# godhj93/bayesian-torch

Hardware: AMD Instinct MI355X
Metric: MC-samples/sec (forward+KL), Bayesian-ResNet18 CIFAR batch=128 (higher is better)
Workload: dtype f32 (bf16x3 split operands, 6 product terms, f32 accumulate); 1 GPU; cfg3: Bayesian-ResNet18 via dnn_to_bnn (Conv2dReparameterization), CIFAR 3x32x32, batch=128; samples_per_launch=32, batch=128, rng=on-chip philox, parallelism=mc1, output_stage=bn+relu+residual (+ the stem max-pool) folded into the conv kernels, launch=hip graph replay

## Files before the change

### bayesian_torch_amd/csrc/bt_fused_fwd.h

```cpp
#pragma once
#include <type_traits>

#include "bt_api_internal.h"

namespace bt {

typedef float f32x16 __attribute__((ext_vector_type(16)));

constexpr int kBK = 36;
constexpr int kMaxTaps = 128;
#ifndef BT_STAMPS
#define BT_STAMPS 0
#endif
constexpr bool kStamps = BT_STAMPS != 0;
constexpr int kThreads = 512;
constexpr int kProducers = 256;

struct FwdArgs {
  const float *x, *mu_w, *rho_w, *mu_b, *rho_b, *pmu_w, *psig_w, *pmu_b, *psig_b;
  const float *mu_pk, *sig_pk;
  const float *eps_w, *eps_b, *sign_in, *sign_out;
  float* out;
  float* kl_out;
  double* slots;
  unsigned* counter;
  long long x_sample_stride, x_elems, out_elems, w_elems;
  int B, Ci, H, W, Co, KH, KW, SH, SW, PH, PW, DH, DW, G;
  int Ho, Wo, HoWo, M, K, Cig, Cog, S, T, HW;
  int n_tiles, m_tiles, total_blocks;
  int t_NI, t_R, t_Wt, n_bt, n_rt, n_ct;
  int patch_ok;
  int x_cvec;
  int x_rows;
  int pixel_major, mt_per_pixel;
  int w_vec, x_vec;
  int do_kl, kl_slices;
  uint32_t seed_lo, seed_hi, call, layer_id, sample0;
  const uint32_t* call_base;
  const float *ep_scale, *ep_shift, *ep_res;
  long long ep_res_stride;
  int ep_relu;
  int ep_pool, ep_Hp, ep_Wp;
  int out_vec4;
  int bn32;
  unsigned long long* dbg;
  uint32_t inv_m_tiles, inv_S, inv_n_tiles, inv_n_bt, inv_n_ct, inv_rw, inv_wt, inv_kw;
  int x_flat;
  int row_taps;
  float* sk_scratch;
  unsigned* sk_tickets;
  long long sk_scratch_bytes;
  int sk_nsl, sk_ks, sk_cpt;
  int sk_kh0, sk_nh, sk_kw0, sk_nw;
  int d_tap;
};

__device__ __forceinline__ int xcd_remap(int orig, int n) {
  const int q = n >> 3, r = n & 7, xcd = orig & 7, i = orig >> 3;
  return (xcd < r ? xcd * (q + 1) : r * (q + 1) + (xcd - r) * q) + i;
}

__host__ __device__ inline int row_chunks(int x_lo, int x_hi, int W, int* xa_out) {
  const int xa = x_lo & ~3;
  int n = ((x_hi - xa) >> 2) + 1;
  if (n > 1 && xa + 4 * (n - 1) >= W && xa + 4 <= 0) --n;
  *xa_out = xa;
  return n;
}

template <int BM, bool FLIP = false>
constexpr int x_words() {
  return kBK * ((FLIP && BM > 128 ? 160 : BM <= 256 ? BM : 320) + 1);
}

template <int BN, int BM, bool FLIP>
constexpr int fused_lds_bytes() {
  return (2 * (FLIP ? 2 : 1) * (kBK * (BN + 1) + x_words<BM, FLIP>()) + kMaxTaps * 4 + 24 + 8 + 80) * 4;
}

__device__ __forceinline__ double block_sum_all(double v, double* scratch) {
  v = wave_sum(v);
  const int lane = threadIdx.x & 63, w = threadIdx.x >> 6;
  __syncthreads();
  if (lane == 0) scratch[w] = v;
  __syncthreads();
  double t = 0.0;
  if (threadIdx.x == 0)
// ... 710 lines not shown
```

### bayesian_torch_amd/csrc/bt_fused_split.hip

```cpp
#include <atomic>
#include <stdlib.h>
#include <string.h>

#include "bt_fused_split_quad.h"
#include "bt_fused_split_direct.h"
#include "bt_fused_split_skinny.h"
#include "bt_fused_split_host.h"

namespace bt {

static std::atomic<int> g_contraction{-1};
int contraction_mode() {
  int m = g_contraction.load(std::memory_order_relaxed);
  if (m < 0) {
    const char* e = getenv("BT_CONTRACTION");
    m = !e ? 0 : (!strcmp(e, "f32") ? 1 : !strcmp(e, "bf16x2") ? 2 : 0);
    g_contraction.store(m, std::memory_order_relaxed);
  }
  return m;
}

template <int BM, int NP, int NPW, int XM, int BN = 64>
static int launch_split_cfg(FwdArgs& a, hipStream_t stream) {
  constexpr int lds = split_lds_bytes<BN, BM, NP>();
// ... 6 lines not shown
    if (hipFuncSetAttribute(reinterpret_cast<const void*>(kern), hipFuncAttributeMaxDynamicSharedMemorySize, lds) != hipSuccess)
      return set_error(BT_ERR_HIP_BASE, "fused forward (split): cannot raise the dynamic LDS limit");
    flags[dev] = true;
  }
  char nm[160];
  snprintf(nm, sizeof(nm), "fused_split_kernel<%d,%d,bf16x%d,%d terms,npw=%d,xm=%d>", BN, BM, NP, NP == 3 ? 6 : 3, NPW, XM);
  note_kernel(nm);
  split_fill_inverses(a);
  hipLaunchKernelGGL(kern, dim3((unsigned)a.total_blocks), dim3(256 + 64 * NPW), lds, stream, a);
  return check_launch("fused forward (split)");
}

template <int BM, int NPW>
static int launch_split_xm(FwdArgs& a, int mode, int xm, hipStream_t stream) {
  if (mode == 2) return launch_split_cfg<BM, 2, NPW, 0>(a, stream);
  if constexpr (BM == 128) {
    if (a.bn32) {
      if (xm == 1) return launch_split_cfg<BM, 3, NPW, 1, 32>(a, stream);
      if (xm == 2) return launch_split_cfg<BM, 3, NPW, 2, 32>(a, stream);
      return launch_split_cfg<BM, 3, NPW, 0, 32>(a, stream);
    }
    if (xm == 1) return launch_split_cfg<BM, 3, NPW, 1>(a, stream);
    if (xm == 2) return launch_split_cfg<BM, 3, NPW, 2>(a, stream);
  } else {
    if (xm == 3) return launch_split_cfg<BM, 3, NPW, 3>(a, stream);
    if (xm == 4) return launch_split_cfg<BM, 3, NPW, 4>(a, stream);
    if constexpr (BM == 256) {
      if (xm == 2) return launch_split_cfg<BM, 3, 8, 2>(a, stream);
    }
  }
  return launch_split_cfg<BM, 3, NPW, 0>(a, stream);
}

template <bool POOL>
static int launch_quad_cfg(FwdArgs& a, int mode, hipStream_t stream) {
  constexpr int lds = split_lds_bytes<64, 512, 3>();
  auto launch = [&](auto kern, const char* nm) -> int {
    static bool flags[2][64] = {};
    int dev = 0;
    if (hipGetDevice(&dev) != hipSuccess || dev < 0 || dev >= 64) return set_error(BT_ERR_HIP_BASE, "fused forward (split): hipGetDevice failed");
    if (!flags[mode == 2][dev]) {
      if (hipFuncSetAttribute(reinterpret_cast<const void*>(kern), hipFuncAttributeMaxDynamicSharedMemorySize, lds) != hipSuccess)
        return set_error(BT_ERR_HIP_BASE, "fused forward (split): cannot raise the dynamic LDS limit");
      flags[mode == 2][dev] = true;
    }
    note_kernel(nm);
    split_fill_inverses(a);
    hipLaunchKernelGGL(kern, dim3((unsigned)a.total_blocks), dim3(512), lds, stream, a);
    return check_launch("fused forward (split, quad)");
  };
  return launch(fused_split_quad_kernel<3, POOL>, POOL ? "fused_split_quad_kernel<64,512,bf16x3,6 terms,pool=1>" : "fused_split_quad_kernel<64,512,bf16x3,6 terms,pool=0>");
}

static int launch_quad(FwdArgs& a, int mode, hipStream_t stream) {
  if (a.pixel_major || a.T > 64 || !a.out_vec4 || a.HoWo < 2 || a.Wo > 512) return 1;
  int nh, nw, dys, dxs;
  tap_window(a.KH, a.DH, a.SH, a.PH, a.H, a.Ho, false, &nh, &dys);
  tap_window(a.KW, a.DW, a.SW, a.PW, a.W, a.Wo, false, &nw, &dxs);
  constexpr long long XCAP = kQuadXBytes / 24;
  const long long PWt = (long long)(a.Wo - 1) * (dxs ? a.SW : 1) + dxs + 1;
  int NI, R;
  long long tiles_per_sample;
  if (a.HoWo <= 512) {
    const long long PHt = (long long)(a.Ho - 1) * (dys ? a.SH : 1) + dys + 1;
    NI = 512 / a.HoWo, R = a.Ho;
    if (NI > a.B) NI = a.B;
    while (NI > 1 && NI * PHt * PWt > XCAP) --NI;
    if (NI * PHt * PWt > XCAP) return 1;
    tiles_per_sample = (a.B + NI - 1) / NI;
  } else {
    if (a.ep_pool) return 1;
    NI = 1, R = 512 / a.Wo;
    while (R > 1 && ((long long)(R - 1) * (dys ? a.SH : 1) + dys + 1) * PWt > XCAP) --R;
    if (((long long)(R - 1) * (dys ? a.SH : 1) + dys + 1) * PWt > XCAP) return 1;
    tiles_per_sample = (long long)a.B * ((a.Ho + R - 1) / R);
  }
  if ((double)a.M / ((double)tiles_per_sample * 512) < 0.75) return 1;
  if (a.ep_pool) {
    const int Wp = a.ep_Wp;
    if ((Wp & (Wp - 1)) != 0 || Wp < 4 || Wp > 16 || a.ep_res) return 1;
  }
  a.n_tiles = (a.Cog + 63) / 64;
  a.t_NI = NI, a.t_R = R, a.t_Wt = a.Wo, a.n_bt = (a.B + NI - 1) / NI, a.n_rt = (a.Ho + R - 1) / R, a.n_ct = 1, a.m_tiles = a.n_bt * a.n_rt;
  const long long total = (long long)a.G * a.n_tiles * a.S * a.m_tiles;
  if (total <= 0 || total > 0x7FFFFFFFll) return 1;
  a.total_blocks = (int)total;
  a.kl_slices = total < 256 ? (int)total : 256;
  return a.ep_pool ? launch_quad_cfg<true>(a, mode, stream) : launch_quad_cfg<false>(a, mode, stream);
}

static std::atomic<int> g_bn32{-2};
static std::atomic<int> g_direct_off{0};
static int launch_direct(FwdArgs& a, hipStream_t stream) {
  if (g_direct_off.load(std::memory_order_relaxed)) return 1;
  if (a.ep_pool) return 1;
  if (a.KH == 1 && a.KW == 1 && a.PH == 0 && a.PW == 0) {
    a.d_tap = 0;
  } else if (a.H == 1 && a.W == 1 && a.Ho == 1 && a.Wo == 1 && a.PH % a.DH == 0 && a.PW % a.DW == 0 && a.PH / a.DH < a.KH && a.PW / a.DW < a.KW) {
    a.d_tap = (a.PH / a.DH) * a.KW + a.PW / a.DW;
  } else {
    return 1;
  }
  const bool resident = a.Cig <= kDirectMaxK;
  if ((a.Cig & 63) || (!resident && ((a.Cig % (16 * kDirectChunk)) || a.M < 4096)) || a.M < 64) return 1;
  a.n_tiles = (a.Cog + 63) / 64;
  const long long pairs = (long long)a.G * a.n_tiles * a.S;
  const int nsub = (a.M + 63) / 64;
  static const int wg_env = [] { const char* e = getenv("BT_DIRECT_WGS"); const int v = e ? atoi(e) : 0; return v > 0 ? v : 0; }();
  static const int n_cu = [] { int dev = 0, v = 0; if (hipGetDevice(&dev) != hipSuccess || hipDeviceGetAttribute(&v, hipDeviceAttributeMultiprocessorCount, dev) != hipSuccess || v <= 0) v = 256; return v; }();
  const int wg_target = wg_env ? wg_env : !resident ? n_cu : (a.SH > 1 || a.SW > 1) ? 16 * n_cu : 4 * n_cu;
  long long chunks = (wg_target + pairs - 1) / pairs;
  if (chunks > nsub / 64) chunks = nsub / 64;
  if (chunks < 1) {
    chunks = (256 + pairs - 1) / pairs;
    if (chunks > nsub / 4) chunks = nsub / 4;
    if (chunks < 1) chunks = 1;
  }
  int spc = (int)((nsub + chunks - 1) / chunks);
  if (!resident) spc = (spc + 7) & ~7;
  chunks = (nsub + spc - 1) / spc;
// ... 190 lines not shown
```

### bayesian_torch_amd/csrc/bt_fused_split_host.h

```cpp
#pragma once
#include <stdlib.h>

#include "bt_fused_split.h"

namespace bt {

int contraction_mode();

static inline uint32_t inv_u32(long long d, long long nmax) {
  if (d <= 1 || nmax < 0 || (unsigned long long)nmax * (unsigned long long)d >= (1ull << 32)) return 0u;
  return (uint32_t)(((1ull << 32) + (unsigned long long)d - 1ull) / (unsigned long long)d);
}
static inline void split_fill_inverses(FwdArgs& a) {
  static const bool off = getenv("BT_NO_HOST_INV") != nullptr;
  if (off) {
    a.inv_m_tiles = a.inv_S = a.inv_n_tiles = a.inv_n_bt = a.inv_n_ct = a.inv_rw = a.inv_wt = a.inv_kw = 0u;
    return;
  }
  const long long tb = a.total_blocks;
  a.inv_m_tiles = inv_u32(a.m_tiles, tb);
  a.inv_S = inv_u32(a.S, tb);
  a.inv_n_tiles = inv_u32(a.n_tiles, tb);
  a.inv_n_bt = inv_u32(a.n_bt, a.m_tiles);
  a.inv_n_ct = inv_u32(a.n_ct, a.m_tiles);
  a.inv_rw = inv_u32((long long)a.t_R * a.t_Wt, 1024);
  a.inv_wt = inv_u32(a.t_Wt, 1024);
  a.inv_kw = inv_u32(a.KW, 64);
}

static void tap_window(int K, int D, int S, int P, int In, int Out, bool per_pixel, int* n_act, int* extent, int* n_min = nullptr) {
  int best_n = 0, best_ext = 0, least_n = 1 << 30;
  if (per_pixel) {
    for (int o = 0; o < Out; ++o) {
      int lo = 1 << 30, hi = -1, n = 0;
      for (int k = 0; k < K; ++k)
        if ((unsigned)(o * S - P + k * D) < (unsigned)In) lo = k * D < lo ? k * D : lo, hi = k * D > hi ? k * D : hi, ++n;
      if (n > best_n) best_n = n;
      if (n < least_n) least_n = n;
      if (hi - lo > best_ext) best_ext = hi - lo;
    }
    if (n_min) *n_min = least_n;
  } else {
    int lo = 1 << 30, hi = -1;
    for (int k = 0; k < K; ++k) {
      const int l = P - k * D, c = l > 0 ? (l + S - 1) / S : 0;
      if (c < Out && c * S - l < In) lo = k * D < lo ? k * D : lo, hi = k * D > hi ? k * D : hi, ++best_n;
    }
    best_ext = hi >= lo ? hi - lo : 0;
  }
  *n_act = best_n, *extent = best_ext;
}

static int split_axis_kept(int K, int D, int S, int P, int In, int Out, int* gs_out) {
  int lo = 1 << 30, hi = -1;
  for (int k = 0; k < K; ++k) {
    const int l = P - k * D, c = l > 0 ? (l + S - 1) / S : 0;
    if (c < Out && c * S - l < In) lo = k * D < lo ? k * D : lo, hi = k * D > hi ? k * D : hi;
  }
  *gs_out = 1;
  if (hi < 0) return 0;
// ... 69 lines not shown
```

### bayesian_torch_amd/csrc/bt_fused_split_quad.h

```cpp
#pragma once
#include "bt_fused_split.h"

namespace bt {

constexpr int kQuadXBytes = 2 * split_x_bytes<512, 3>();
constexpr int kQuadXBytesFlip = 38400;
template <bool FLIP>
constexpr int quad_lds_bytes() { return 2 * split_w_bytes<64, 3, FLIP>() + (FLIP ? kQuadXBytesFlip : kQuadXBytes) + kSplitMiscBytes; }

template <int NP, bool POOL, bool FLIP = false>
__global__ __launch_bounds__(512) void fused_split_quad_kernel(const FwdArgs a) {
  constexpr int BN = 64, BM = FLIP ? 256 : 512, kProducers = 256, kThreadsAll = 512, STEPS = kSplitSteps, TPS = 4 * STEPS;
  constexpr int CWM = FLIP ? 2 : 4, CWN = 4 / CWM, WTM = BM / CWM, TN = BN / CWN / 32, TM = WTM / 32, NOP = FLIP ? 2 : 1;
  constexpr int PBQ = 8 * NP;
  constexpr int W_BYTES = split_w_bytes<BN, NP, FLIP>(), W_OP = W_BYTES / NOP, XQ_BYTES = FLIP ? kQuadXBytesFlip : kQuadXBytes;
  constexpr int W_STEP = 2 * NP * BN * 16, W_HALF = NP * BN * 16, W_PIECE = BN * 16;
  constexpr int SROWS = BN, SROW = BM + 4;
  static_assert(!FLIP || NP == 3, "Flipout: the exact split");
  static_assert((4 * BN + NOP * SROWS * SROW) * 4 <= 2 * W_BYTES + XQ_BYTES, "output staging fits the operand buffers");

  extern __shared__ __attribute__((aligned(16))) char smem_c[];
  char* const wbuf = smem_c;
  char* const xq = smem_c + 2 * W_BYTES;
  float* const smem = reinterpret_cast<float*>(smem_c);
  int4* const taptab = reinterpret_cast<int4*>(smem_c + 2 * W_BYTES + XQ_BYTES);
  double* const red = reinterpret_cast<double*>(smem_c + 2 * W_BYTES + XQ_BYTES + kMaxTaps * 16);
  int* const misc = reinterpret_cast<int*>(red + 12);
  int* const eofftab = reinterpret_cast<int*>(taptab + 64);
  (void)red;

  const int tid = threadIdx.x, lane = tid & 63, wave = tid >> 6;
  unsigned long long* const dbg_ = kStamps ? a.dbg : nullptr;
  if (dbg_ && dbg_[201] && tid == 0) {
    dbg_[256 + 4 * blockIdx.x] = __builtin_amdgcn_s_memrealtime();
    dbg_[256 + 4 * blockIdx.x + 2] = __builtin_amdgcn_s_memtime();
  }
  const bool stamp0 = dbg_ && blockIdx.x == 0 && tid == 0;
  if (stamp0) dbg_[210] = __builtin_amdgcn_s_memtime();
  const bool producer = wave >= 4;
  const int ptid = producer ? tid - 256 : tid;
  const int li = lane & 31, lh = lane >> 5;
  const int wm = wave & (CWM - 1), wn = (wave & 3) / CWM;

  int L = __builtin_amdgcn_readfirstlane(xcd_remap(blockIdx.x, a.total_blocks));
  int Lq = udiv_inv(L, a.m_tiles, a.inv_m_tiles);
  const int mt = __builtin_amdgcn_readfirstlane(L - Lq * a.m_tiles);
  L = Lq, Lq = udiv_inv(L, a.S, a.inv_S);
  const int s = __builtin_amdgcn_readfirstlane(L - Lq * a.S);
  L = Lq, Lq = udiv_inv(L, a.n_tiles, a.inv_n_tiles);
  const int nt = __builtin_amdgcn_readfirstlane(L - Lq * a.n_tiles);
  const int g = __builtin_amdgcn_readfirstlane(Lq);
  const int n0 = nt * BN;
  const int t_NI = a.t_NI, t_R = a.t_R, t_Wt = a.t_Wt, RW = t_R * t_Wt, Mt = t_NI * RW;
  const int trest = udiv_inv(mt, a.n_bt, a.inv_n_bt);
  const int bt = __builtin_amdgcn_readfirstlane(mt - trest * a.n_bt);
  const int rt = __builtin_amdgcn_readfirstlane(udiv_inv(trest, a.n_ct, a.inv_n_ct)), ct = __builtin_amdgcn_readfirstlane(trest - rt * a.n_ct);
  const int b0 = bt * t_NI, r0 = rt * t_R, w0 = ct * t_Wt;
  const uint32_t inv_rw = RW > 1 ? (a.inv_rw ? a.inv_rw : inv32(RW)) : 0u;
  const uint32_t inv_wt = t_Wt > 1 ? (a.inv_wt ? a.inv_wt : inv32(t_Wt)) : 0u;
  auto col_decode = [&](int ml, int& b, int& ho, int& wo) -> bool {
    const int img = RW == 1 ? ml : (int)__umulhi((uint32_t)ml, inv_rw);
    const int rem = ml - img * RW;
    const int r = t_Wt == 1 ? rem : (int)__umulhi((uint32_t)rem, inv_wt);
    b = b0 + img, ho = r0 + r, wo = w0 + (rem - r * t_Wt);
    return ml < Mt && b < a.B && ho < a.Ho && wo < a.Wo;
  };
  const uint32_t sample = a.sample0 + (uint32_t)s;
  const int T = a.T, Cig = a.Cig;

  RngKey key_w;
  key_w.seed_lo = a.seed_lo;
  key_w.seed_hi = a.seed_hi;
  key_w.call = a.call + (a.call_base ? __builtin_nontemporal_load(a.call_base) : 0u);
  key_w.layer_tensor = layer_tensor_word(a.layer_id, 0);
  uint32_t skey_in = 0, skey_out = 0;
  if constexpr (FLIP) {
    RngKey ks = key_w;
    ks.layer_tensor = layer_tensor_word(a.layer_id, 2);
    skey_in = sign_stream_key(ks, sample);
    ks.layer_tensor = layer_tensor_word(a.layer_id, 3);
    skey_out = sign_stream_key(ks, sample);
// ... 114 lines not shown
          m = nmax(m, iny ? cd.y : -INFINITY);
        }
        if (relu) m = m < 0.f ? 0.f : m;
        if (ok) oplane[py * Wp + px] = m;
      }
    }
  };

  auto combine_flip = [&](int t0) {
    constexpr int QROW = BM / 4, RSTEP = kThreadsAll / QROW, NIT = SROWS / RSTEP;
    static_assert(kThreadsAll % QROW == 0 && SROWS % RSTEP == 0, "a thread keeps its pixel quad");
    float* const stage = smem + 4 * BN;
    const int m4 = t0 % QROW, row0 = t0 / QROW;
    int bq, hq, wq;
    const bool mok = col_decode(4 * m4, bq, hq, wq);
    const int HoWo_ = a.Ho * a.Wo;
    const uint32_t obase = mok ? (uint32_t)(((bq * a.Co + g * a.Cog + n0 + row0) * a.Ho + hq) * a.Wo + wq) : 0u;
#pragma unroll
    for (int k = 0; k < NIT; ++k) {
      const int row = row0 + k * RSTEP;
      float* const p0 = stage + row * SROW + 4 * m4;
      float4 v = *reinterpret_cast<const float4*>(p0);
      const float4 d = *reinterpret_cast<const float4*>(p0 + SROWS * SROW);
      const uint32_t oi = obase + (uint32_t)(k * RSTEP * HoWo_);
      const float sc = osc[row], sh = osh[row];
      v.x = __fadd_rn(__fmul_rn(__fadd_rn(v.x, __fmul_rn(d.x, hash_sign(skey_out, oi))), sc), sh);
      v.y = __fadd_rn(__fmul_rn(__fadd_rn(v.y, __fmul_rn(d.y, hash_sign(skey_out, oi + 1u))), sc), sh);
      v.z = __fadd_rn(__fmul_rn(__fadd_rn(v.z, __fmul_rn(d.z, hash_sign(skey_out, oi + 2u))), sc), sh);
      v.w = __fadd_rn(__fmul_rn(__fadd_rn(v.w, __fmul_rn(d.w, hash_sign(skey_out, oi + 3u))), sc), sh);
      *reinterpret_cast<float4*>(p0) = v;
    }
  };

  {
    const uint32_t inv_pimg = PIMG > 1 ? inv32(PIMG) : 0u;
    const uint32_t inv_pw = PWt > 1 ? inv32(PWt) : 0u;
    const int HWb = 4 * a.HW;
    constexpr int XB = 4;
    for (int i0 = 0; i0 * kThreadsAll < PCH; i0 += XB) {
      float xv[XB][4];
      int pos_[XB];
      uint32_t xoff_[XB];
#pragma unroll
      for (int k = 0; k < XB; ++k) {
        const int pos = tid + kThreadsAll * (i0 + k);
        pos_[k] = pos;
        const int pp = pos < PCH ? pos : 0;
        const int img = PIMG == 1 ? pp : (int)__umulhi((uint32_t)pp, inv_pimg);
        const int rem = pp - img * PIMG;
        const int yy = PWt == 1 ? rem : (int)__umulhi((uint32_t)rem, inv_pw);
        const int xx = rem - yy * PWt;
        const int b = b0 + img, y = y_lo + yy * gs_h, x = x_lo + xx * gs_w;
        const bool ok = pos < PCH && b < a.B && (unsigned)y < (unsigned)a.H && (unsigned)x < (unsigned)a.W;
        const uint32_t off = ok ? (uint32_t)(4 * ((b * a.Ci + g * Cig) * a.HW + y * a.W + x)) : kOOB;
        xoff_[k] = ok ? off : 0u;
#pragma unroll
        for (int c = 0; c < 4; ++c) xv[k][c] = ldf(r_x, (ok && c < Cig) ? off + (uint32_t)(c * HWb) : kOOB);
      }
#pragma unroll
      for (int k = 0; k < XB; ++k) {
        if (pos_[k] < PCH) {
          uint32_t ph[4], pm[4], pl[4];
#pragma unroll
          for (int c = 0; c < 4; ++c) split_pieces(xv[k][c], ph[c], pm[c], pl[c]);
          if constexpr (FLIP) {
            uint32_t bits = 0;
#pragma unroll
            for (int c = 0; c < 3; ++c)
              bits |= (__float_as_uint(hash_sign(skey_in, (xoff_[k] >> 2) + (uint32_t)(c * a.HW))) >> 31) << (16 + c);
            ph[3] = bits;
          }
          char* const dst = xq + pos_[k] * PBQ;
          *reinterpret_cast<uint2*>(dst) = make_uint2(pack_hi16(ph[1], ph[0]), pack_hi16(ph[3], ph[2]));
          *reinterpret_cast<uint2*>(dst + 8) = make_uint2(pack_hi16(pm[1], pm[0]), pack_hi16(pm[3], pm[2]));
          if constexpr (NP == 3) *reinterpret_cast<uint2*>(dst + 16) = make_uint2(pack_hi16(pl[1], pl[0]), pack_hi16(pl[3], pl[2]));
        }
      }
    }
  }
  if (stamp0) dbg_[212] = __builtin_amdgcn_s_memtime();
  if (producer) {
    constexpr int UMAX = (BN * TPS + kProducers - 1) / kProducers;
    int l_off[UMAX];
    uint32_t u_co[UMAX];
#pragma unroll
    for (int i = 0; i < UMAX; ++i) {
      const int u = ptid + kProducers * i, n = u & (BN - 1), q = u >> 6;
      const int st_ = q >> 2, hf = (q >> 1) & 1, sub = q & 1;
      const int co_g = n0 + n;
      u_co[i] = co_g < a.Cog ? (uint32_t)(g * a.Cog + co_g) : 0xFFFFFFFFu;
      l_off[i] = st_ * W_STEP + hf * W_HALF + (n ^ ((2 * st_ + hf) & 7)) * 16 + sub * 8;
    }
    float4 mu[UMAX], rs[UMAX];
    uint32_t ue[UMAX];
    auto load_w = [&](int st) {
#pragma unroll
      for (int i = 0; i < UMAX; ++i) {
        const int ai = st * TPS + ((ptid + kProducers * i) >> 6);
        const bool in = ai < nA && u_co[i] != 0xFFFFFFFFu;
        const int tap = taptab[ai < nA ? ai : 0].w;
        ue[i] = in ? (u_co[i] * (uint32_t)T + (uint32_t)tap) * 4u : (kOOB >> 2);
        mu[i] = ldf4(r_mu, in ? 4u * ue[i] : kOOB), rs[i] = ldf4(r_rs, in ? 4u * ue[i] : kOOB);
      }
    };
    if (NS > 0) load_w(0);
    for (int st = 0; st <= NS; ++st) {
      if (st < NS) {
        char* const Wt = wbuf + (st & 1) * W_BYTES;
        float ep[UMAX][4];
#pragma unroll
        for (int i = 0; i < UMAX; ++i) philox_normal4(key_w, sample, ue[i] >> 2, ep[i]);
#pragma unroll
        for (int i = 0; i < UMAX; ++i) {
          const float m4[4] = {mu[i].x, mu[i].y, mu[i].z, mu[i].w}, s4[4] = {rs[i].x, rs[i].y, rs[i].z, rs[i].w};
          uint32_t wh[4], wm_[4], wl[4];
#pragma unroll
          for (int j = 0; j < 4; ++j)
            split_pieces(FLIP ? m4[j] : __fadd_rn(m4[j], __fmul_rn(s4[j], ep[i][j])), wh[j], wm_[j], wl[j]);
          char* const dst = Wt + l_off[i];
          *reinterpret_cast<uint2*>(dst) = make_uint2(pack_hi16(wh[1], wh[0]), pack_hi16(wh[3], wh[2]));
          *reinterpret_cast<uint2*>(dst + W_PIECE) = make_uint2(pack_hi16(wm_[1], wm_[0]), pack_hi16(wm_[3], wm_[2]));
          if constexpr (NP == 3) *reinterpret_cast<uint2*>(dst + 2 * W_PIECE) = make_uint2(pack_hi16(wl[1], wl[0]), pack_hi16(wl[3], wl[2]));
          if constexpr (FLIP) {
#pragma unroll
            for (int j = 0; j < 4; ++j) split_pieces(__fmul_rn(s4[j], ep[i][j]), wh[j], wm_[j], wl[j]);
            *reinterpret_cast<uint2*>(dst + W_OP) = make_uint2(pack_hi16(wh[1], wh[0]), pack_hi16(wh[3], wh[2]));
            *reinterpret_cast<uint2*>(dst + W_OP + W_PIECE) = make_uint2(pack_hi16(wm_[1], wm_[0]), pack_hi16(wm_[3], wm_[2]));
            *reinterpret_cast<uint2*>(dst + W_OP + 2 * W_PIECE) = make_uint2(pack_hi16(wl[1], wl[0]), pack_hi16(wl[3], wl[2]));
          }
        }
        if (st + 1 < NS) load_w(st + 1);
      }
      __syncthreads();
    }
    if (ptid < BN) {
      float bv = 0.f;
      const int co_g = n0 + ptid;
      if (a.mu_b && co_g < a.Cog) {
        const int co = g * a.Cog + co_g;
        RngKey kb = key_w;
        kb.layer_tensor = layer_tensor_word(a.layer_id, 1);
        float z[4];
        philox_normal4(kb, sample, (uint32_t)(co >> 2), z);
        const int sel = co & 3;
        const float e = sel == 0 ? z[0] : sel == 1 ? z[1] : sel == 2 ? z[2] : z[3];
        const float dl = __fmul_rn(softplus(a.rho_b[co]), e);
        bv = FLIP ? a.mu_b[co] : __fadd_rn(a.mu_b[co], dl);
        if constexpr (FLIP) bias1[ptid] = dl;
      } else if constexpr (FLIP) {
        bias1[ptid] = 0.f;
      }
      bias0[ptid] = bv;
      const bool cv = a.ep_scale && co_g < a.Cog;
      const int cs = cv ? g * a.Cog + co_g : 0;
      const float sc = a.ep_scale ? a.ep_scale[cs] : 1.f, sh = a.ep_shift ? a.ep_shift[cs] : 0.f;
      osc[ptid] = cv ? sc : 1.f;
      osh[ptid] = cv ? sh : 0.f;
    }
    __syncthreads();
    __syncthreads();
    if constexpr (FLIP) {
      combine_flip(tid);
      __syncthreads();
    }
    if constexpr (POOL) readout_pool(wave);
    else readout_quads(tid);
  } else {
    long long kl_i = 0, kl_hi = 0;
    double kl_acc = 0.0;
    bool kl_v4 = false;
    if (kl_block) {
      long long chunk = (a.w_elems + a.kl_slices - 1) / a.kl_slices;
      chunk = (chunk + 3) & ~3ll;
      const long long lo = (long long)blockIdx.x * chunk;
      kl_hi = (lo + chunk < a.w_elems) ? lo + chunk : a.w_elems;
      kl_v4 = ((((uintptr_t)a.mu_w | (uintptr_t)a.rho_w | (uintptr_t)a.pmu_w | (uintptr_t)a.psig_w) & 15u) == 0);
      kl_i = lo + 4ll * ptid;
    }
    auto kl_group = [&]() {
      if (!(kl_v4 && kl_i + 3 < kl_hi)) return false;
      const float4 m4 = *reinterpret_cast<const float4*>(a.mu_w + kl_i), r4 = *reinterpret_cast<const float4*>(a.rho_w + kl_i);
      const float4 p4 = *reinterpret_cast<const float4*>(a.pmu_w + kl_i), q4 = *reinterpret_cast<const float4*>(a.psig_w + kl_i);
      const float t0 = kl_term(m4.x, softplus(r4.x), p4.x, q4.x) + kl_term(m4.y, softplus(r4.y), p4.y, q4.y);
      const float t1 = kl_term(m4.z, softplus(r4.z), p4.z, q4.z) + kl_term(m4.w, softplus(r4.w), p4.w, q4.w);
      kl_acc += (double)t0 + (double)t1;
      kl_i += 1024;
      return true;
    };
    auto kl_finish = [&]() {
      while (kl_group()) {}
      for (; kl_i < kl_hi; kl_i += 1024)
        for (int j = 0; j < 4; ++j)
          if (kl_i + j < kl_hi) kl_acc += (double)kl_term(a.mu_w[kl_i + j], softplus(a.rho_w[kl_i + j]), a.pmu_w[kl_i + j], a.psig_w[kl_i + j]);
      const double wsum = wave_sum(kl_acc);
      if (lane == 0) __hip_atomic_store(&a.slots[(int)blockIdx.x * 4 + wave], wsum, __ATOMIC_RELAXED, __HIP_MEMORY_SCOPE_AGENT);
      asm volatile("s_waitcnt vmcnt(0)" ::: "memory");
    };
    auto kl_ticket = [&]() {
      const int nslots = 4 * a.kl_slices;
// ... 7 lines not shown
        if (a.mu_b)
          for (int c = lane; c < a.Co; c += 64) bt_ += (double)kl_term(a.mu_b[c], softplus(a.rho_b[c]), a.pmu_b[c], a.psig_b[c]);
        bt_ = wave_sum(bt_);
        if (lane == 0) {
          float kl = (float)(t / (double)a.w_elems);
          if (a.mu_b) kl += (float)(bt_ / (double)a.Co);
          a.kl_out[0] = kl;
          __hip_atomic_store(a.counter, 0u, __ATOMIC_RELAXED, __HIP_MEMORY_SCOPE_AGENT);
        }
      }
    };
    int colq[TM];
#pragma unroll
    for (int j = 0; j < TM; ++j) {
      const int ml = wm * WTM + j * 32 + li;
      int b, ho, wo;
      const bool live = col_decode(ml, b, ho, wo);
      colq[j] = live ? ((b - b0) * PIMG + (ho - r0) * ps_h * PWt + (wo - w0) * ps_w) * PBQ : 0;
    }
    int wlq[STEPS];
#pragma unroll
    for (int q = 0; q < STEPS; ++q) wlq[q] = lh * W_HALF + (li ^ ((2 * q + lh) & 7)) * 16 + wn * TN * 32 * 16;

    f32x16 acc[NOP][TN][TM];
#pragma unroll
    for (int o = 0; o < NOP; ++o)
#pragma unroll
      for (int i = 0; i < TN; ++i)
#pragma unroll
        for (int j = 0; j < TM; ++j)
#pragma unroll
          for (int r = 0; r < 16; ++r) acc[o][i][j][r] = 0.f;

    __syncthreads();
    if (stamp0) dbg_[0] = __builtin_amdgcn_s_memtime();
    for (int st = 0; st < NS; ++st) {
      if (stamp0) dbg_[2 + 2 * st] = __builtin_amdgcn_s_memtime();
      const char* const Wt = wbuf + (st & 1) * W_BYTES;
      const int left = nA - st * TPS, nstep = left >= TPS ? STEPS : (left + 3) >> 2;
      int eA[STEPS], eB[STEPS];
#pragma unroll
      for (int q = 0; q < STEPS; ++q) eA[q] = eofftab[st * TPS + 4 * q + 2 * lh], eB[q] = eofftab[st * TPS + 4 * q + 2 * lh + 1];
      bf16x8 wf[2][NOP][TN][NP];
      uint2 xlo[2][NP], xhi[2][NP];
      auto read_w = [&](int q) {
#pragma unroll
        for (int o = 0; o < NOP; ++o)
#pragma unroll
          for (int i = 0; i < TN; ++i)
#pragma unroll
            for (int p = 0; p < NP; ++p)
              wf[q & 1][o][i][p] = *reinterpret_cast<const bf16x8*>(Wt + o * W_OP + wlq[q] + q * W_STEP + p * W_PIECE + i * 32 * 16);
      };
      auto read_x = [&](int u) {
        const int q = u / TM, j = u % TM;
#pragma unroll
        for (int p = 0; p < NP; ++p) {
          xlo[u & 1][p] = *reinterpret_cast<const uint2*>(xq + colq[j] + eA[q] + 8 * p);
          xhi[u & 1][p] = *reinterpret_cast<const uint2*>(xq + colq[j] + eB[q] + 8 * p);
        }
      };
      read_w(0);
      read_x(0);
#pragma unroll
      for (int q = 0; q < STEPS; ++q) {
        if (q < nstep) {
#pragma unroll
          for (int j = 0; j < TM; ++j) {
            const int u = q * TM + j;
            if (j + 1 < TM) {
              read_x(u + 1);
// ... 6 lines not shown
            __builtin_amdgcn_sched_barrier(0);
            bf16x8 xf[NP];
#pragma unroll
            for (int p = 0; p < NP; ++p) xf[p] = __builtin_bit_cast(bf16x8, make_uint4(xlo[u & 1][p].x, xlo[u & 1][p].y, xhi[u & 1][p].x, xhi[u & 1][p].y));
#pragma unroll
            for (int o = 0; o < NOP; ++o) {
              if (o == 1) {
                const uint32_t mA = xlo[u & 1][0].y, mB = xhi[u & 1][0].y;
                const uint4 mk = make_uint4(((mA & 0x10000u) >> 1) | ((mA & 0x20000u) << 14), (mA & 0x40000u) >> 3,
                                            ((mB & 0x10000u) >> 1) | ((mB & 0x20000u) << 14), (mB & 0x40000u) >> 3);
#pragma unroll
                for (int p = 0; p < NP; ++p) {
                  uint4 t = __builtin_bit_cast(uint4, xf[p]);
                  t.x ^= mk.x, t.y ^= mk.y, t.z ^= mk.z, t.w ^= mk.w;
                  xf[p] = __builtin_bit_cast(bf16x8, t);
                }
              }
#pragma unroll
              for (int i = 0; i < TN; ++i) {
                acc[o][i][j] = __builtin_amdgcn_mfma_f32_32x32x16_bf16(xf[0], wf[q & 1][o][i][0], acc[o][i][j], 0, 0, 0);
                acc[o][i][j] = __builtin_amdgcn_mfma_f32_32x32x16_bf16(xf[0], wf[q & 1][o][i][1], acc[o][i][j], 0, 0, 0);
                acc[o][i][j] = __builtin_amdgcn_mfma_f32_32x32x16_bf16(xf[1], wf[q & 1][o][i][0], acc[o][i][j], 0, 0, 0);
                if constexpr (NP == 3) {
                  acc[o][i][j] = __builtin_amdgcn_mfma_f32_32x32x16_bf16(xf[0], wf[q & 1][o][i][2], acc[o][i][j], 0, 0, 0);
                  acc[o][i][j] = __builtin_amdgcn_mfma_f32_32x32x16_bf16(xf[1], wf[q & 1][o][i][1], acc[o][i][j], 0, 0, 0);
                  acc[o][i][j] = __builtin_amdgcn_mfma_f32_32x32x16_bf16(xf[2], wf[q & 1][o][i][0], acc[o][i][j], 0, 0, 0);
                }
              }
            }
            __builtin_amdgcn_sched_barrier(0);
          }
        }
      }
      if (stamp0) dbg_[2 + 2 * st + 1] = __builtin_amdgcn_s_memtime();
      if (kl_block) kl_group();
      __syncthreads();
    }
    if (kl_block) kl_finish();
    if (stamp0) dbg_[1] = __builtin_amdgcn_s_memtime();
    __syncthreads();
    if (kl_block && wave == 0) kl_ticket();

    float* const stage = smem + 4 * BN;
    float bsv[TN], scv[TN], shv[TN], b1v[TN];
#pragma unroll
    for (int i = 0; i < TN; ++i) {
      const int co_l = (wn * TN + i) * 32 + li;
      bsv[i] = bias0[co_l], scv[i] = osc[co_l], shv[i] = osh[co_l];
      b1v[i] = FLIP ? bias1[co_l] : 0.f;
    }
#pragma unroll
    for (int i = 0; i < TN; ++i) {
      float* const srow = stage + ((wn * TN + i) * 32 + li) * SROW + wm * WTM + 4 * lh;
#pragma unroll
      for (int j = 0; j < TM; ++j) {
#pragma unroll
        for (int q = 0; q < 4; ++q) {
          float v[4];
          if constexpr (FLIP) {
#pragma unroll
            for (int e = 0; e < 4; ++e) v[e] = __fadd_rn(acc[0][i][j][4 * q + e], bsv[i]);
            *reinterpret_cast<float4*>(srow + j * 32 + 8 * q) = make_float4(v[0], v[1], v[2], v[3]);
#pragma unroll
            for (int e = 0; e < 4; ++e) v[e] = __fadd_rn(acc[NOP - 1][i][j][4 * q + e], b1v[i]);
            *reinterpret_cast<float4*>(srow + SROWS * SROW + j * 32 + 8 * q) = make_float4(v[0], v[1], v[2], v[3]);
          } else {
#pragma unroll
            for (int e = 0; e < 4; ++e) v[e] = __fadd_rn(__fmul_rn(__fadd_rn(acc[0][i][j][4 * q + e], bsv[i]), scv[i]), shv[i]);
            *reinterpret_cast<float4*>(srow + j * 32 + 8 * q) = make_float4(v[0], v[1], v[2], v[3]);
          }
        }
      }
    }
    __syncthreads();
    if constexpr (FLIP) {
      combine_flip(tid);
      __syncthreads();
    }
    if (stamp0) dbg_[121] = __builtin_amdgcn_s_memtime();
    if constexpr (POOL) readout_pool(wave);
    else readout_quads(tid);
    if (stamp0) dbg_[126] = __builtin_amdgcn_s_memtime();
  }
  if (dbg_ && dbg_[201] && tid == 0) {
    dbg_[256 + 4 * blockIdx.x + 1] = __builtin_amdgcn_s_memrealtime();
    dbg_[256 + 4 * blockIdx.x + 2] = __builtin_amdgcn_s_memtime() - dbg_[256 + 4 * blockIdx.x + 2];
  }
}

}
```

Measured before the change: 18210 MC-samples/s.

## Walk several MC samples per block in pooled quad conv, reusing staged input

For the pooled stem-style quad conv (16x16 output, 8x8 pool, two images per tile), each block now processes up to spw MC samples in sequence. The input tile stays resident in LDS while the producer waves draw each sample's weights in a continuous double-buffered pipeline across sample boundaries. The max-pool epilogue is done in registers, using lane shuffles and a small LDS row exchange between waves, instead of the staging readout. This cuts redundant input staging and per-block setup, and reduces block count. The cost is less parallelism across the grid, more kernel complexity and a narrow shape-specific path.

```diff
diff --git a/bayesian_torch_amd/csrc/bt_fused_fwd.h b/bayesian_torch_amd/csrc/bt_fused_fwd.h
--- a/bayesian_torch_amd/csrc/bt_fused_fwd.h
+++ b/bayesian_torch_amd/csrc/bt_fused_fwd.h
@@ -53,6 +53,8 @@
   int sk_nsl, sk_ks, sk_cpt;
   int sk_kh0, sk_nh, sk_kw0, sk_nw;
   int d_tap;
+  int spw, n_sg;
+  uint32_t inv_n_sg;
 };
 
 __device__ __forceinline__ int xcd_remap(int orig, int n) {
diff --git a/bayesian_torch_amd/csrc/bt_fused_split.hip b/bayesian_torch_amd/csrc/bt_fused_split.hip
--- a/bayesian_torch_amd/csrc/bt_fused_split.hip
+++ b/bayesian_torch_amd/csrc/bt_fused_split.hip
@@ -62,7 +62,7 @@
   return launch_split_cfg<BM, 3, NPW, 0>(a, stream);
 }
 
-template <bool POOL>
+template <bool POOL, bool WALK = false>
 static int launch_quad_cfg(FwdArgs& a, int mode, hipStream_t stream) {
   constexpr int lds = split_lds_bytes<64, 512, 3>();
   auto launch = [&](auto kern, const char* nm) -> int {
@@ -79,7 +79,28 @@
     hipLaunchKernelGGL(kern, dim3((unsigned)a.total_blocks), dim3(512), lds, stream, a);
     return check_launch("fused forward (split, quad)");
   };
+  if constexpr (WALK) return launch(fused_split_quad_kernel<3, true, false, true>, "fused_split_quad_kernel<64,512,bf16x3,6 terms,pool=1,walk>");
   return launch(fused_split_quad_kernel<3, POOL>, POOL ? "fused_split_quad_kernel<64,512,bf16x3,6 terms,pool=1>" : "fused_split_quad_kernel<64,512,bf16x3,6 terms,pool=0>");
+}
+
+static int quad_spw(const FwdArgs& a, long long tiles) {
+  if (!a.ep_pool || a.x_sample_stride != 0 || a.S < 2 || a.Ho != 16 || a.Wo != 16 || a.t_NI != 2 || a.ep_Hp != 8 || a.ep_Wp != 8) return 0;
+  int nd[2] = {};
+  tap_window(a.KH, a.DH, a.SH, a.PH, a.H, a.Ho, false, &nd[0], &nd[1]);
+  int nw, dxs;
+  tap_window(a.KW, a.DW, a.SW, a.PW, a.W, a.Wo, false, &nw, &dxs);
+  const long long PHt = 15ll * (nd[1] ? a.SH : 1) + nd[1] + 1, PWt = 15ll * (dxs ? a.SW : 1) + dxs + 1;
+  if (2 * PHt * PWt * 24 + kWalkBytes > kQuadXBytes) return 0;
+  static int n_cu[64] = {};
+  int dev = 0;
+  if (hipGetDevice(&dev) != hipSuccess || dev < 0 || dev >= 64) return 0;
+  if (!n_cu[dev] && hipDeviceGetAttribute(&n_cu[dev], hipDeviceAttributeMultiprocessorCount, dev) != hipSuccess) n_cu[dev] = 0;
+  const long long fill = n_cu[dev] > 256 ? n_cu[dev] : 256;
+  const char* e = getenv("BT_QUAD_SPW");
+  const int cap = e ? atoi(e) : 8;
+  for (int spw = 8; spw >= 2; spw >>= 1)
+    if (spw <= cap && spw <= a.S && tiles * ((a.S + spw - 1) / spw) >= fill) return spw;
+  return 0;
 }
 
 static int launch_quad(FwdArgs& a, int mode, hipStream_t stream) {
@@ -112,10 +133,14 @@
   }
   a.n_tiles = (a.Cog + 63) / 64;
   a.t_NI = NI, a.t_R = R, a.t_Wt = a.Wo, a.n_bt = (a.B + NI - 1) / NI, a.n_rt = (a.Ho + R - 1) / R, a.n_ct = 1, a.m_tiles = a.n_bt * a.n_rt;
-  const long long total = (long long)a.G * a.n_tiles * a.S * a.m_tiles;
+  const long long tiles = (long long)a.G * a.n_tiles * a.m_tiles;
+  const int spw = quad_spw(a, tiles);
+  a.spw = spw ? spw : 1, a.n_sg = (a.S + a.spw - 1) / a.spw;
+  const long long total = tiles * a.n_sg;
   if (total <= 0 || total > 0x7FFFFFFFll) return 1;
   a.total_blocks = (int)total;
   a.kl_slices = total < 256 ? (int)total : 256;
+  if (spw) return launch_quad_cfg<true, true>(a, mode, stream);
   return a.ep_pool ? launch_quad_cfg<true>(a, mode, stream) : launch_quad_cfg<false>(a, mode, stream);
 }
 
diff --git a/bayesian_torch_amd/csrc/bt_fused_split_host.h b/bayesian_torch_amd/csrc/bt_fused_split_host.h
--- a/bayesian_torch_amd/csrc/bt_fused_split_host.h
+++ b/bayesian_torch_amd/csrc/bt_fused_split_host.h
@@ -14,7 +14,7 @@
 static inline void split_fill_inverses(FwdArgs& a) {
   static const bool off = getenv("BT_NO_HOST_INV") != nullptr;
   if (off) {
-    a.inv_m_tiles = a.inv_S = a.inv_n_tiles = a.inv_n_bt = a.inv_n_ct = a.inv_rw = a.inv_wt = a.inv_kw = 0u;
+    a.inv_m_tiles = a.inv_S = a.inv_n_tiles = a.inv_n_bt = a.inv_n_ct = a.inv_rw = a.inv_wt = a.inv_kw = a.inv_n_sg = 0u;
     return;
   }
   const long long tb = a.total_blocks;
@@ -26,6 +26,7 @@
   a.inv_rw = inv_u32((long long)a.t_R * a.t_Wt, 1024);
   a.inv_wt = inv_u32(a.t_Wt, 1024);
   a.inv_kw = inv_u32(a.KW, 64);
+  a.inv_n_sg = inv_u32(a.n_sg, tb);
 }
 
 static void tap_window(int K, int D, int S, int P, int In, int Out, bool per_pixel, int* n_act, int* extent, int* n_min = nullptr) {
diff --git a/bayesian_torch_amd/csrc/bt_fused_split_quad.h b/bayesian_torch_amd/csrc/bt_fused_split_quad.h
--- a/bayesian_torch_amd/csrc/bt_fused_split_quad.h
+++ b/bayesian_torch_amd/csrc/bt_fused_split_quad.h
@@ -8,7 +8,10 @@
 template <bool FLIP>
 constexpr int quad_lds_bytes() { return 2 * split_w_bytes<64, 3, FLIP>() + (FLIP ? kQuadXBytesFlip : kQuadXBytes) + kSplitMiscBytes; }
 
-template <int NP, bool POOL, bool FLIP = false>
+constexpr int kWalkRowBytes = 2 * 64 * 16 * 4;
+constexpr int kWalkBytes = 2 * kWalkRowBytes + 2 * 3 * 64 * 4;
+
+template <int NP, bool POOL, bool FLIP = false, bool WALK = false>
 __global__ __launch_bounds__(512) void fused_split_quad_kernel(const FwdArgs a) {
   constexpr int BN = 64, BM = FLIP ? 256 : 512, kProducers = 256, kThreadsAll = 512, STEPS = kSplitSteps, TPS = 4 * STEPS;
   constexpr int CWM = FLIP ? 2 : 4, CWN = 4 / CWM, WTM = BM / CWM, TN = BN / CWN / 32, TM = WTM / 32, NOP = FLIP ? 2 : 1;
@@ -17,11 +20,14 @@
   constexpr int W_STEP = 2 * NP * BN * 16, W_HALF = NP * BN * 16, W_PIECE = BN * 16;
   constexpr int SROWS = BN, SROW = BM + 4;
   static_assert(!FLIP || NP == 3, "Flipout: the exact split");
+  static_assert(!WALK || (POOL && !FLIP && CWM == 4 && TN == 2 && TM == 4), "the walk: Reparameterization, pooled, 4 x 128-pixel consumer waves");
   static_assert((4 * BN + NOP * SROWS * SROW) * 4 <= 2 * W_BYTES + XQ_BYTES, "output staging fits the operand buffers");
 
   extern __shared__ __attribute__((aligned(16))) char smem_c[];
   char* const wbuf = smem_c;
   char* const xq = smem_c + 2 * W_BYTES;
+  float* const wrow = reinterpret_cast<float*>(xq + XQ_BYTES - kWalkBytes);
+  float* const wcon = wrow + 2 * kWalkRowBytes / 4;
   float* const smem = reinterpret_cast<float*>(smem_c);
   int4* const taptab = reinterpret_cast<int4*>(smem_c + 2 * W_BYTES + XQ_BYTES);
   double* const red = reinterpret_cast<double*>(smem_c + 2 * W_BYTES + XQ_BYTES + kMaxTaps * 16);
@@ -45,8 +51,9 @@
   int L = __builtin_amdgcn_readfirstlane(xcd_remap(blockIdx.x, a.total_blocks));
   int Lq = udiv_inv(L, a.m_tiles, a.inv_m_tiles);
   const int mt = __builtin_amdgcn_readfirstlane(L - Lq * a.m_tiles);
-  L = Lq, Lq = udiv_inv(L, a.S, a.inv_S);
-  const int s = __builtin_amdgcn_readfirstlane(L - Lq * a.S);
+  const int SD = WALK ? a.n_sg : a.S;
+  L = Lq, Lq = udiv_inv(L, SD, WALK ? a.inv_n_sg : a.inv_S);
+  const int s = __builtin_amdgcn_readfirstlane((L - Lq * SD) * (WALK ? a.spw : 1));
   L = Lq, Lq = udiv_inv(L, a.n_tiles, a.inv_n_tiles);
   const int nt = __builtin_amdgcn_readfirstlane(L - Lq * a.n_tiles);
   const int g = __builtin_amdgcn_readfirstlane(Lq);
@@ -227,6 +234,31 @@
     }
   };
 
+  constexpr int UMAX = (BN * TPS + kProducers - 1) / kProducers;
+  int l_off[UMAX];
+  uint32_t u_co[UMAX];
+#pragma unroll
+  for (int i = 0; i < UMAX; ++i) {
+    const int u = ptid + kProducers * i, n = u & (BN - 1), q = u >> 6;
+    const int st_ = q >> 2, hf = (q >> 1) & 1, sub = q & 1;
+    const int co_g = n0 + n;
+    u_co[i] = co_g < a.Cog ? (uint32_t)(g * a.Cog + co_g) : 0xFFFFFFFFu;
+    l_off[i] = st_ * W_STEP + hf * W_HALF + (n ^ ((2 * st_ + hf) & 7)) * 16 + sub * 8;
+  }
+  float4 mu[UMAX], rs[UMAX];
+  uint32_t ue[UMAX];
+  auto load_w = [&](int st) {
+#pragma unroll
+    for (int i = 0; i < UMAX; ++i) {
+      const int ai = st * TPS + ((ptid + kProducers * i) >> 6);
+      const bool in = ai < nA && u_co[i] != 0xFFFFFFFFu;
+      const int tap = taptab[ai < nA ? ai : 0].w;
+      ue[i] = in ? (u_co[i] * (uint32_t)T + (uint32_t)tap) * 4u : (kOOB >> 2);
+      mu[i] = ldf4(r_mu, in ? 4u * ue[i] : kOOB), rs[i] = ldf4(r_rs, in ? 4u * ue[i] : kOOB);
+    }
+  };
+  if (!FLIP && producer && NS > 0) load_w(0);
+
   {
     const uint32_t inv_pimg = PIMG > 1 ? inv32(PIMG) : 0u;
     const uint32_t inv_pw = PWt > 1 ? inv32(PWt) : 0u;
@@ -275,60 +307,31 @@
   }
   if (stamp0) dbg_[212] = __builtin_amdgcn_s_memtime();
   if (producer) {
-    constexpr int UMAX = (BN * TPS + kProducers - 1) / kProducers;
-    int l_off[UMAX];
-    uint32_t u_co[UMAX];
-#pragma unroll
-    for (int i = 0; i < UMAX; ++i) {
-      const int u = ptid + kProducers * i, n = u & (BN - 1), q = u >> 6;
-      const int st_ = q >> 2, hf = (q >> 1) & 1, sub = q & 1;
-      const int co_g = n0 + n;
-      u_co[i] = co_g < a.Cog ? (uint32_t)(g * a.Cog + co_g) : 0xFFFFFFFFu;
-      l_off[i] = st_ * W_STEP + hf * W_HALF + (n ^ ((2 * st_ + hf) & 7)) * 16 + sub * 8;
-    }
-    float4 mu[UMAX], rs[UMAX];
-    uint32_t ue[UMAX];
-    auto load_w = [&](int st) {
+    auto draw_stage = [&](uint32_t smp, char* const Wt) {
+      float ep[UMAX][4];
+#pragma unroll
+      for (int i = 0; i < UMAX; ++i) philox_normal4(key_w, smp, ue[i] >> 2, ep[i]);
 #pragma unroll
       for (int i = 0; i < UMAX; ++i) {
-        const int ai = st * TPS + ((ptid + kProducers * i) >> 6);
-        const bool in = ai < nA && u_co[i] != 0xFFFFFFFFu;
-        const int tap = taptab[ai < nA ? ai : 0].w;
-        ue[i] = in ? (u_co[i] * (uint32_t)T + (uint32_t)tap) * 4u : (kOOB >> 2);
-        mu[i] = ldf4(r_mu, in ? 4u * ue[i] : kOOB), rs[i] = ldf4(r_rs, in ? 4u * ue[i] : kOOB);
+        const float m4[4] = {mu[i].x, mu[i].y, mu[i].z, mu[i].w}, s4[4] = {rs[i].x, rs[i].y, rs[i].z, rs[i].w};
+        uint32_t wh[4], wm_[4], wl[4];
+#pragma unroll
+        for (int j = 0; j < 4; ++j)
+          split_pieces(FLIP ? m4[j] : __fadd_rn(m4[j], __fmul_rn(s4[j], ep[i][j])), wh[j], wm_[j], wl[j]);
+        char* const dst = Wt + l_off[i];
+        *reinterpret_cast<uint2*>(dst) = make_uint2(pack_hi16(wh[1], wh[0]), pack_hi16(wh[3], wh[2]));
+        *reinterpret_cast<uint2*>(dst + W_PIECE) = make_uint2(pack_hi16(wm_[1], wm_[0]), pack_hi16(wm_[3], wm_[2]));
+        if constexpr (NP == 3) *reinterpret_cast<uint2*>(dst + 2 * W_PIECE) = make_uint2(pack_hi16(wl[1], wl[0]), pack_hi16(wl[3], wl[2]));
+        if constexpr (FLIP) {
+#pragma unroll
+          for (int j = 0; j < 4; ++j) split_pieces(__fmul_rn(s4[j], ep[i][j]), wh[j], wm_[j], wl[j]);
+          *reinterpret_cast<uint2*>(dst + W_OP) = make_uint2(pack_hi16(wh[1], wh[0]), pack_hi16(wh[3], wh[2]));
+          *reinterpret_cast<uint2*>(dst + W_OP + W_PIECE) = make_uint2(pack_hi16(wm_[1], wm_[0]), pack_hi16(wm_[3], wm_[2]));
+          *reinterpret_cast<uint2*>(dst + W_OP + 2 * W_PIECE) = make_uint2(pack_hi16(wl[1], wl[0]), pack_hi16(wl[3], wl[2]));
+        }
       }
     };
-    if (NS > 0) load_w(0);
-    for (int st = 0; st <= NS; ++st) {
-      if (st < NS) {
-        char* const Wt = wbuf + (st & 1) * W_BYTES;
-        float ep[UMAX][4];
-#pragma unroll
-        for (int i = 0; i < UMAX; ++i) philox_normal4(key_w, sample, ue[i] >> 2, ep[i]);
-#pragma unroll
-        for (int i = 0; i < UMAX; ++i) {
-          const float m4[4] = {mu[i].x, mu[i].y, mu[i].z, mu[i].w}, s4[4] = {rs[i].x, rs[i].y, rs[i].z, rs[i].w};
-          uint32_t wh[4], wm_[4], wl[4];
-#pragma unroll
-          for (int j = 0; j < 4; ++j)
-            split_pieces(FLIP ? m4[j] : __fadd_rn(m4[j], __fmul_rn(s4[j], ep[i][j])), wh[j], wm_[j], wl[j]);
-          char* const dst = Wt + l_off[i];
-          *reinterpret_cast<uint2*>(dst) = make_uint2(pack_hi16(wh[1], wh[0]), pack_hi16(wh[3], wh[2]));
-          *reinterpret_cast<uint2*>(dst + W_PIECE) = make_uint2(pack_hi16(wm_[1], wm_[0]), pack_hi16(wm_[3], wm_[2]));
-          if constexpr (NP == 3) *reinterpret_cast<uint2*>(dst + 2 * W_PIECE) = make_uint2(pack_hi16(wl[1], wl[0]), pack_hi16(wl[3], wl[2]));
-          if constexpr (FLIP) {
-#pragma unroll
-            for (int j = 0; j < 4; ++j) split_pieces(__fmul_rn(s4[j], ep[i][j]), wh[j], wm_[j], wl[j]);
-            *reinterpret_cast<uint2*>(dst + W_OP) = make_uint2(pack_hi16(wh[1], wh[0]), pack_hi16(wh[3], wh[2]));
-            *reinterpret_cast<uint2*>(dst + W_OP + W_PIECE) = make_uint2(pack_hi16(wm_[1], wm_[0]), pack_hi16(wm_[3], wm_[2]));
-            *reinterpret_cast<uint2*>(dst + W_OP + 2 * W_PIECE) = make_uint2(pack_hi16(wl[1], wl[0]), pack_hi16(wl[3], wl[2]));
-          }
-        }
-        if (st + 1 < NS) load_w(st + 1);
-      }
-      __syncthreads();
-    }
-    if (ptid < BN) {
+    auto bias_consts = [&](uint32_t smp, float* const b0p, float* const b1p, float* const scp, float* const shp) {
       float bv = 0.f;
       const int co_g = n0 + ptid;
       if (a.mu_b && co_g < a.Cog) {
@@ -336,22 +339,49 @@
         RngKey kb = key_w;
         kb.layer_tensor = layer_tensor_word(a.layer_id, 1);
         float z[4];
-        philox_normal4(kb, sample, (uint32_t)(co >> 2), z);
+        philox_normal4(kb, smp, (uint32_t)(co >> 2), z);
         const int sel = co & 3;
         const float e = sel == 0 ? z[0] : sel == 1 ? z[1] : sel == 2 ? z[2] : z[3];
         const float dl = __fmul_rn(softplus(a.rho_b[co]), e);
         bv = FLIP ? a.mu_b[co] : __fadd_rn(a.mu_b[co], dl);
-        if constexpr (FLIP) bias1[ptid] = dl;
+        if constexpr (FLIP) b1p[ptid] = dl;
       } else if constexpr (FLIP) {
-        bias1[ptid] = 0.f;
-      }
-      bias0[ptid] = bv;
+        b1p[ptid] = 0.f;
+      }
+      b0p[ptid] = bv;
       const bool cv = a.ep_scale && co_g < a.Cog;
       const int cs = cv ? g * a.Cog + co_g : 0;
       const float sc = a.ep_scale ? a.ep_scale[cs] : 1.f, sh = a.ep_shift ? a.ep_shift[cs] : 0.f;
-      osc[ptid] = cv ? sc : 1.f;
-      osh[ptid] = cv ? sh : 0.f;
-    }
+      scp[ptid] = cv ? sc : 1.f;
+      shp[ptid] = cv ? sh : 0.f;
+    };
+    if constexpr (WALK) {
+      const int nsw = min(a.spw, a.S - s), NSE = NS > 0 ? NS : 1;
+      int G = 0;
+      for (int k = 0; k < nsw; ++k) {
+        const uint32_t smp = sample + (uint32_t)k;
+        float* const cs_ = wcon + (k & 1) * 3 * BN;
+        for (int st = 0; st < NSE; ++st, ++G) {
+          if (st < NS) {
+            draw_stage(smp, wbuf + (G & 1) * W_BYTES);
+            if (st + 1 < NS) load_w(st + 1);
+            else if (k + 1 < nsw) load_w(0);
+          }
+          if (st == 0 && ptid < BN) bias_consts(smp, cs_, cs_, cs_ + BN, cs_ + 2 * BN);
+          __syncthreads();
+        }
+      }
+      __syncthreads();
+    } else {
+    if (FLIP && NS > 0) load_w(0);
+    for (int st = 0; st <= NS; ++st) {
+      if (st < NS) {
+        draw_stage(sample, wbuf + (st & 1) * W_BYTES);
+        if (st + 1 < NS) load_w(st + 1);
+      }
+      __syncthreads();
+    }
+    if (ptid < BN) bias_consts(sample, bias0, bias1, osc, osh);
     __syncthreads();
     __syncthreads();
     if constexpr (FLIP) {
@@ -360,6 +390,7 @@
     }
     if constexpr (POOL) readout_pool(wave);
     else readout_quads(tid);
+    }
   } else {
     long long kl_i = 0, kl_hi = 0;
     double kl_acc = 0.0;
@@ -433,11 +464,7 @@
 #pragma unroll
           for (int r = 0; r < 16; ++r) acc[o][i][j][r] = 0.f;
 
-    __syncthreads();
-    if (stamp0) dbg_[0] = __builtin_amdgcn_s_memtime();
-    for (int st = 0; st < NS; ++st) {
-      if (stamp0) dbg_[2 + 2 * st] = __builtin_amdgcn_s_memtime();
-      const char* const Wt = wbuf + (st & 1) * W_BYTES;
+    auto run_stage = [&](int st, const char* const Wt) {
       const int left = nA - st * TPS, nstep = left >= TPS ? STEPS : (left + 3) >> 2;
       int eA[STEPS], eB[STEPS];
 #pragma unroll
@@ -510,6 +537,101 @@
           }
         }
       }
+    };
+    if constexpr (WALK) {
+      const int nsw = min(a.spw, a.S - s), NSE = NS > 0 ? NS : 1;
+      const bool odd = (wm & 1) != 0;
+      const int bimg = b0 + (wm >> 1);
+      auto nmax = [](float m, float v) { return (v > m || v != v) ? v : m; };
+      __syncthreads();
+      if (stamp0) dbg_[0] = __builtin_amdgcn_s_memtime();
+      int G = 0;
+      for (int k = 0; k < nsw; ++k) {
+        if (k > 0) {
+#pragma unroll
+          for (int i = 0; i < TN; ++i)
+#pragma unroll
+            for (int j = 0; j < TM; ++j)
+#pragma unroll
+              for (int r = 0; r < 16; ++r) acc[0][i][j][r] = 0.f;
+        }
+        const float* const cs_ = wcon + (k & 1) * 3 * BN;
+        float* const xrow = wrow + (k & 1) * (kWalkRowBytes / 4) + (wm >> 1) * (BN * 16);
+        for (int st = 0; st < NSE; ++st, ++G) {
+          if (stamp0 && G < 48) dbg_[2 + 2 * G] = __builtin_amdgcn_s_memtime();
+          if (st < NS) run_stage(st, wbuf + (G & 1) * W_BYTES);
+          if (stamp0 && G < 48) dbg_[2 + 2 * G + 1] = __builtin_amdgcn_s_memtime();
+          if (st + 1 == NSE) {
+#pragma unroll
+            for (int i = 0; i < TN; ++i) {
+              const int co_l = i * 32 + li;
+              const float bsv = cs_[co_l], scv = cs_[BN + co_l], shv = cs_[2 * BN + co_l];
+#pragma unroll
+              for (int j = 0; j < TM; ++j)
+#pragma unroll
+                for (int r = 0; r < 16; ++r) acc[0][i][j][r] = __fadd_rn(__fmul_rn(__fadd_rn(acc[0][i][j][r], bsv), scv), shv);
+              if (!odd) {
+#pragma unroll
+                for (int h = 0; h < 2; ++h)
+                  *reinterpret_cast<float4*>(xrow + co_l * 16 + 8 * h + 4 * lh) =
+                      make_float4(acc[0][i][3][8 + 4 * h], acc[0][i][3][9 + 4 * h], acc[0][i][3][10 + 4 * h], acc[0][i][3][11 + 4 * h]);
+              }
+            }
+            if (kl_block) {
+              if (k + 1 == nsw) kl_finish();
+              else kl_group();
+            }
+          } else if (kl_block) {
+            kl_group();
+          }
+          __syncthreads();
+        }
+        float* const out_k = a.out + (long long)(s + k) * a.out_elems;
+#pragma unroll
+        for (int i = 0; i < TN; ++i) {
+          const int co_l = i * 32 + li;
+          const bool ok = bimg < a.B && n0 + co_l < a.Cog;
+          float* const oplane = out_k + (ok ? (bimg * a.Co + g * a.Cog + n0 + co_l) * 64 : 0) + 32 * (wm & 1);
+          float top[2][4];
+#pragma unroll
+          for (int h = 0; h < 2; ++h) {
+            const float4 t = odd ? *reinterpret_cast<const float4*>(xrow + co_l * 16 + 8 * h + 4 * lh) : make_float4(-INFINITY, -INFINITY, -INFINITY, -INFINITY);
+            top[h][0] = t.x, top[h][1] = t.y, top[h][2] = t.z, top[h][3] = t.w;
+          }
+          auto val = [&](int r, int h, int e) -> float { return r < 0 ? top[h][e] : acc[0][i][r >> 1][4 * (2 * (r & 1) + h) + e]; };
+#pragma unroll
+          for (int py = 0; py < 4; ++py) {
+            float m[2][2] = {{-INFINITY, -INFINITY}, {-INFINITY, -INFINITY}};
+#pragma unroll
+            for (int dy = 0; dy < 3; ++dy) {
+              const int r = 2 * py - 1 + dy;
+              const float x0 = __shfl_xor(val(r, 0, 3), 32, 64), x1 = __shfl_xor(val(r, 1, 3), 32, 64);
+#pragma unroll
+              for (int h = 0; h < 2; ++h) {
+                const float l0 = lh ? (h ? x1 : x0) : (h ? x0 : -INFINITY);
+                m[h][0] = nmax(nmax(nmax(m[h][0], l0), val(r, h, 0)), val(r, h, 1));
+                m[h][1] = nmax(nmax(nmax(m[h][1], val(r, h, 1)), val(r, h, 2)), val(r, h, 3));
+              }
+            }
+#pragma unroll
+            for (int h = 0; h < 2; ++h) {
+              if (relu) {
+                m[h][0] = m[h][0] < 0.f ? 0.f : m[h][0];
+                m[h][1] = m[h][1] < 0.f ? 0.f : m[h][1];
+              }
+              if (ok) *reinterpret_cast<float2*>(oplane + 8 * py + 4 * h + 2 * lh) = make_float2(m[h][0], m[h][1]);
+            }
+          }
+        }
+      }
+      if (stamp0) dbg_[1] = __builtin_amdgcn_s_memtime();
+      if (kl_block && wave == 0) kl_ticket();
+    } else {
+    __syncthreads();
+    if (stamp0) dbg_[0] = __builtin_amdgcn_s_memtime();
+    for (int st = 0; st < NS; ++st) {
+      if (stamp0) dbg_[2 + 2 * st] = __builtin_amdgcn_s_memtime();
+      run_stage(st, wbuf + (st & 1) * W_BYTES);
       if (stamp0) dbg_[2 + 2 * st + 1] = __builtin_amdgcn_s_memtime();
       if (kl_block) kl_group();
       __syncthreads();
@@ -559,6 +681,7 @@
     if constexpr (POOL) readout_pool(wave);
     else readout_quads(tid);
     if (stamp0) dbg_[126] = __builtin_amdgcn_s_memtime();
+    }
   }
   if (dbg_ && dbg_[201] && tid == 0) {
     dbg_[256 + 4 * blockIdx.x + 1] = __builtin_amdgcn_s_memrealtime();
```

Measured after the change: 18720 MC-samples/s (median of 6 runs). 1.03x the previous value.
